# NVlabs/FB-BEV

Hardware: AMD Instinct MI355X
Metric: multi-cam samples/sec (forward view transformation: lift + voxel ranking + bev_pool_v2) (higher is better)
Workload: dtype f32

## Files before the change

fb_bev_amd/csrc/capi.hip:

```cpp
#include <stdio.h>
#include <stdlib.h>
#include <mutex>
#include "rt.h"
#include "pool_kernels.h"
#include "pool_bwd_kernels.h"
#include "rank_kernels.h"
#include "sort_kernels.h"
#include "msda_kernels.h"
#include "geom_kernels.h"
#include "da_kernels.h"
#include "history_kernels.h"
#include "norm_kernels.h"
#include "history_conv_kernels.h"
#include "history_fused_kernels.h"
#include "history_conv_x3_kernels.h"
#include "history_fused_x3_kernels.h"
#include "rows_linear_kernels.h"
#include "rows_linear_f32_kernels.h"
#include "da_fused_kernels.h"
#include "da_bwd_planes_kernels.h"
#include "msda_bwd_kernels.h"
#include "conv3d_kernels.h"
#include "det_kernels.h"
#include "occ_kernels.h"
// ... 29 lines not shown
}

extern "C" int fbbev_bev_pool_v2_bwd(int c, int n_intervals, const float* out_grad,
                                     const float* depth, const float* feat,
                                     const int32_t* ranks_depth, const int32_t* ranks_feat,
                                     const int32_t* ranks_bev, const int32_t* interval_starts,
                                     const int32_t* interval_lengths, float* depth_grad,
                                     float* feat_grad, fbbev_stream_t stream_) {
    if (c <= 0 || n_intervals < 0) return FBBEV_E_BADARG;
    if (c > 256) return FBBEV_E_UNSUPPORTED;
    if (n_intervals == 0) return 0;
    if (!out_grad || !depth || !feat || !ranks_depth || !ranks_feat || !ranks_bev ||
        !interval_starts || !interval_lengths || !depth_grad || !feat_grad) return FBBEV_E_BADARG;
    fbbev_rt_stream stream = (fbbev_rt_stream)stream_;
    const long long blocks = ((long long)n_intervals * 64 + 255) / 256;
    const int nch = (c + 63) / 64;
#define FBBEV_BWD(NCH)                                                                             \
    FBBEV_LAUNCH(k_pool_bwd<NCH>, blocks, 256, 0, stream, c, n_intervals, out_grad, depth, feat,   \
                 ranks_depth, ranks_feat, ranks_bev, interval_starts, interval_lengths, depth_grad, \
                 feat_grad)
    switch (nch) {
        case 1: FBBEV_BWD(1); break;
        case 2: FBBEV_BWD(2); break;
        case 3: FBBEV_BWD(3); break;
        default: FBBEV_BWD(4); break;
    }
#undef FBBEV_BWD
    FBBEV_CHECK_LAUNCH();
    return 0;
}

extern "C" int fbbev_lidar_coor(const float* xs, const float* ys, const float* ds, const float* rots,
                                const float* trans, const float* intrins, const float* post_rots,
                                const float* post_trans, const float* bda, int B, int N, int D, int H,
                                int W, float* coor, fbbev_stream_t stream_) {
    if (B <= 0 || N <= 0 || D <= 0 || H <= 0 || W <= 0) return FBBEV_E_BADARG;
    if (!xs || !ys || !ds || !rots || !trans || !intrins || !post_rots || !post_trans || !bda || !coor)
        return FBBEV_E_BADARG;
    const long long dhw = (long long)D * H * W;
    const long long chunks = (dhw + 255) / 256;
    if (chunks * B * N >= (1ll << 31)) return FBBEV_E_UNSUPPORTED;
    fbbev_cam_ptrs g;
    g.xs = xs; g.ys = ys; g.ds = ds; g.rots = rots; g.trans = trans; g.intrins = intrins; g.post_rots = post_rots;
    g.post_trans = post_trans; g.bda = bda; g.N = N; g.D = D; g.H = H; g.W = W;
    FBBEV_LAUNCH(k_lidar_coor, chunks * B * N, 256, 0, (fbbev_rt_stream)stream_, g, (int)chunks, coor);
    FBBEV_CHECK_LAUNCH();
    return 0;
}

extern "C" int fbbev_nchw_to_nhwc(const float* in, float* out, int n_images, int C, int HW, fbbev_stream_t stream_) {
    return fbbev_tokens_from_nchw(in, out, n_images, C, HW, (long long)C * HW, 0, nullptr, 0, stream_);
}

static int tokens_from_nchw_impl(const float* in, float* out, int n_images, int C, int HW, long long out_image_stride,
                                 long long out_offset, const float* bias, int bias_rows, const float* pos_bias,
                                 fbbev_stream_t stream_) {
    if (n_images < 0 || C <= 0 || HW <= 0 || out_offset < 0 || out_image_stride < (long long)C * HW) return FBBEV_E_BADARG;
    if (bias && bias_rows <= 0) return FBBEV_E_BADARG;
    if (n_images == 0) return 0;
    if (!in || !out) return FBBEV_E_BADARG;
    const int tc = (C + 31) / 32, th = (HW + 31) / 32;
    const long long blocks = (long long)n_images * tc * th;
    if (blocks >= (1ll << 31)) return FBBEV_E_UNSUPPORTED;
    FBBEV_LAUNCH(k_nchw_to_nhwc, blocks, 256, 0, (fbbev_rt_stream)stream_, in, out, C, HW, tc, th, out_image_stride,
                 out_offset, bias, bias ? bias_rows : 1, pos_bias);
    FBBEV_CHECK_LAUNCH();
    return 0;
}

extern "C" int fbbev_tokens_from_nchw(const float* in, float* out, int n_images, int C, int HW,
                                      long long out_image_stride, long long out_offset, const float* bias,
                                      int bias_rows, fbbev_stream_t stream_) {
    return tokens_from_nchw_impl(in, out, n_images, C, HW, out_image_stride, out_offset, bias, bias_rows, nullptr, stream_);
}

extern "C" int fbbev_tokens_from_nchw_levels(const float* const* in, const int32_t* hw, int n_levels, float* out, int n_images, int C,
                                             const float* bias, int bias_rows, fbbev_stream_t stream_) {
    if (n_levels <= 0 || n_levels > 8 || n_images < 0 || C <= 0 || !in || !hw) return FBBEV_E_BADARG;
    if (bias && bias_rows <= 0) return FBBEV_E_BADARG;
    if (n_images == 0) return 0;
    if (!out) return FBBEV_E_BADARG;
    fbbev_token_levels lv;
    const int tc = (C + 31) / 32;
    long long start = 0, blocks = 0;
    for (int l = 0; l < 8; ++l) { lv.in[l] = nullptr; lv.out_off[l] = 0; lv.hw[l] = 1; lv.blk0[l] = 0; }
    for (int l = 0; l < n_levels; ++l) {
        if (hw[l] <= 0 || !in[l]) return FBBEV_E_BADARG;
        lv.in[l] = in[l]; lv.hw[l] = hw[l]; lv.out_off[l] = start * C; lv.blk0[l] = (int)blocks;
        start += hw[l];
        blocks += (long long)n_images * tc * ((hw[l] + 31) / 32);
        if (blocks >= (1ll << 31)) return FBBEV_E_UNSUPPORTED;
    }
    lv.blk0[n_levels] = (int)blocks;
    lv.n = n_levels;
    FBBEV_LAUNCH(k_nchw_to_nhwc_levels, blocks, 256, 0, (fbbev_rt_stream)stream_, lv, out, C, tc, start * C, bias, bias ? bias_rows : 1);
    FBBEV_CHECK_LAUNCH();
    return 0;
}

extern "C" int fbbev_tokens_from_nchw_pos(const float* in, float* out, int n_images, int C, int HW, long long out_image_stride,
                                          long long out_offset, const float* pos_bias, fbbev_stream_t stream_) {
    if (!pos_bias) return FBBEV_E_BADARG;
    return tokens_from_nchw_impl(in, out, n_images, C, HW, out_image_stride, out_offset, nullptr, 0, pos_bias, stream_);
}

extern "C" int fbbev_point_sampling(const float* xs, const float* ys, const float* zs, const float* rots,
                                    const float* trans, const float* intrins, const float* post_rots,
                                    const float* post_trans, const float* bda, int B, int N, int Y, int X,
                                    int Za, float ogfH, float ogfW, float* ref_cam, uint8_t* mask,
                                    float* qdepth, fbbev_stream_t stream_) {
    if (B <= 0 || N <= 0 || Y <= 0 || X <= 0 || Za <= 0 || !(ogfH > 0.f) || !(ogfW > 0.f)) return FBBEV_E_BADARG;
    if (!xs || !ys || !zs || !rots || !trans || !intrins || !post_rots || !post_trans || !bda || !ref_cam ||
        !mask || !qdepth) return FBBEV_E_BADARG;
    const long long npts = (long long)Y * X * Za;
    int ppt = 8;
    while (ppt > 1 && (npts + 256 * ppt - 1) / (256 * ppt) * B * N < 1024) ppt >>= 1;
    const long long chunks = (npts + 256 * ppt - 1) / (256 * ppt);
    if (chunks * B * N >= (1ll << 31) || ((uintptr_t)ref_cam & 7) != 0) return FBBEV_E_UNSUPPORTED;
    FBBEV_LAUNCH(k_point_sampling, chunks * B * N, 256, 0, (fbbev_rt_stream)stream_, xs, ys, zs, rots, trans,
                 intrins, post_rots, post_trans, bda, B, N, Y, X, Za, ogfH, ogfW, (int)chunks, ref_cam, mask,
                 qdepth, ppt);
    FBBEV_CHECK_LAUNCH();
    return 0;
}

static inline int key_bits(long long total_voxels) {
    int bits = 1;
    while ((1ll << bits) < total_voxels) ++bits;
    return bits;
}

static const int kSortTile[7] = {2048, 4096, 8192, 12288, 16384, 4096, 8192};
static int sort_variant_for(long long items) {
    for (int v = 0; v < 5; ++v)
        if ((items + kSortTile[v] - 1) / kSortTile[v] <= 256) return v;
    return 6;
}
static const int kIvTile[3] = {1024, 4096, 8192};
static int iv_variant_for(long long items) {
    for (int v = 0; v < 3; ++v)
        if ((items + kIvTile[v] - 1) / kIvTile[v] <= 256) return v;
    return 2;
}

static fbbev_fastdiv make_fastdiv(unsigned int d) {
    fbbev_fastdiv f;
    f.d = d; f.m = 0; f.sh = 0;
    if (d <= 1) { f.d = 1; return f; }
    unsigned int l = 0;
    while ((1ull << l) < d) ++l;
    f.m = (unsigned int)((((1ull << l) - d) << 32) / d + 1);
    f.sh = l - 1;
    return f;
}

struct rank_ws_layout {
    size_t keys_a, keys_t, vals_t, matrix, ctot, chunk_info, boff, hb, total;
    int v0, wgs0;
    int v1, wgs1;
    int vi, wgsi;
};

static rank_ws_layout rank_layout(long long n) {
    rank_ws_layout L;
    L.v0 = sort_variant_for(n);
    L.v1 = sort_variant_for((n + 1) / 2);
    L.vi = iv_variant_for((n + 1) / 2);
    if (const char* env = fbbev_env_str("FBBEV_RANK_SHAPE")) {
        int a = -1, b = -1, c = -1;
        if (sscanf(env, "%d,%d,%d", &a, &b, &c) == 3 && a >= 0 && a < 7 && b >= 0 && b < 7 && c >= 0 && c < 3) {
            L.v0 = a; L.v1 = b; L.vi = c;
        }
    }
    L.wgs0 = (int)((n + kSortTile[L.v0] - 1) / kSortTile[L.v0]);
    L.wgs1 = (int)((n + kSortTile[L.v1] - 1) / kSortTile[L.v1]);
    L.wgsi = (int)((n + kIvTile[L.vi] - 1) / kIvTile[L.vi]);
    size_t off = 0;
    L.keys_a = off; off = align_up(off + (size_t)n * 4, 256);
    L.keys_t = off; off = align_up(off + (size_t)n * 4, 256);
    L.vals_t = off; off = align_up(off + (size_t)n * 4, 256);
    const int rows = L.wgs0 > L.wgs1 ? L.wgs0 : L.wgs1;
    const size_t seg_rows = (size_t)(n / FBBEV_SEG_TILE) + 256 + 1;
    size_t mbytes = (size_t)rows * FBBEV_SORT_MAX_NB * 4;
    if (seg_rows * FBBEV_SEG_NB * 4 > mbytes) mbytes = seg_rows * FBBEV_SEG_NB * 4;
    L.matrix = off; off = align_up(off + mbytes, 256);
    L.ctot = off; off = align_up(off + seg_rows * 4, 256);
    L.chunk_info = off; off = align_up(off + (size_t)L.wgsi * 8, 256);
    const size_t fin_buckets = (size_t)(n < 256 ? n : 256) * FBBEV_SEG_NB;
    L.boff = off; off = align_up(off + (fin_buckets + 1) * 4, 256);
    L.hb = off; off = align_up(off + fin_buckets * 4, 256);
    L.total = off;
    return L;
}

#define FBBEV_SORT_DISPATCH(KERNEL, v, by_waves, grid, stream, ...)                                             \
    do {                                                                                                        \
        switch (v) {                                                                                            \
            case 0: FBBEV_LAUNCH((KERNEL<(by_waves) ? 4 : 256, 8>), grid, 256, 0, stream, __VA_ARGS__); break;   \
            case 1: FBBEV_LAUNCH((KERNEL<(by_waves) ? 16 : 1024, 4>), grid, 1024, 0, stream, __VA_ARGS__); break; \
            case 2: FBBEV_LAUNCH((KERNEL<(by_waves) ? 16 : 1024, 8>), grid, 1024, 0, stream, __VA_ARGS__); break; \
            case 3: FBBEV_LAUNCH((KERNEL<(by_waves) ? 16 : 1024, 12>), grid, 1024, 0, stream, __VA_ARGS__); break; \
            case 5: FBBEV_LAUNCH((KERNEL<(by_waves) ? 8 : 512, 8>), grid, 512, 0, stream, __VA_ARGS__); break;     \
            case 6: FBBEV_LAUNCH((KERNEL<(by_waves) ? 8 : 512, 16>), grid, 512, 0, stream, __VA_ARGS__); break;    \
            default: FBBEV_LAUNCH((KERNEL<(by_waves) ? 16 : 1024, 16>), grid, 1024, 0, stream, __VA_ARGS__); break; \
        }                                                                                                       \
    } while (0)

extern "C" size_t fbbev_rank_workspace_bytes(int64_t n_points) {
    if (n_points <= 0) return 256;
    return rank_layout(n_points).total;
}

static int rank_seg_mode() { FBBEV_KNOB_ONCE(int, m, fbbev_env_int("FBBEV_RANK_SEG", -1)); return m; }
static int rank_finish_mode() { FBBEV_KNOB_ONCE(int, m, fbbev_env_int("FBBEV_RANK_FINISH", -1)); return m; }
static bool rank_finish_auto(int lbits, long long npb, int B) {
    (void)npb; (void)B;
    return lbits >= 2 * FBBEV_SEG_RB;
}

static int rank_build_impl(const float* coor, const fbbev_cam_ptrs* cams, const float* frustum, int B, int N, int D,
                           int H, int W,
                           const float* lower3, const float* interval3, const float* grid_size3,
                           int32_t* ranks_bev, int32_t* ranks_depth, int32_t* ranks_feat,
                           int32_t* interval_starts, int32_t* interval_lengths, int32_t* interval_rank,
                           int32_t* counts, void* workspace, size_t workspace_bytes, fbbev_rt_stream stream,
                           const float* point_depth = nullptr, float depth_thr = 0.f, const int* skip = nullptr) {
    if (B <= 0 || N <= 0 || D <= 0 || H <= 0 || W <= 0) return FBBEV_E_BADARG;
    if (point_depth && cams) return FBBEV_E_UNSUPPORTED;
    if ((!coor && !cams) || !lower3 || !interval3 || !grid_size3 || !ranks_bev || !ranks_depth || !ranks_feat ||
        !interval_starts || !interval_lengths || !counts || !workspace) return FBBEV_E_BADARG;
    const long long n = (long long)B * N * D * H * W;
    if (n >= (1ll << 30)) return FBBEV_E_UNSUPPORTED;
    const rank_ws_layout L = rank_layout(n);
    if (workspace_bytes < L.total) return FBBEV_E_WORKSPACE;
    unsigned char* ws = static_cast<unsigned char*>(workspace);
    unsigned int* keys_a = reinterpret_cast<unsigned int*>(ws + L.keys_a);
    unsigned int* keys_t = reinterpret_cast<unsigned int*>(ws + L.keys_t);
    unsigned int* vals_t = reinterpret_cast<unsigned int*>(ws + L.vals_t);
    int* matrix = reinterpret_cast<int*>(ws + L.matrix);
    int2* chunk_info = reinterpret_cast<int2*>(ws + L.chunk_info);

    fbbev_grid_params gp;
    gp.lx = lower3[0]; gp.ly = lower3[1]; gp.lz = lower3[2];
    gp.ix = interval3[0]; gp.iy = interval3[1]; gp.iz = interval3[2];
    gp.gx = grid_size3[0]; gp.gy = grid_size3[1]; gp.gz = grid_size3[2];
    volatile float zy = gp.gz * gp.gy;
    volatile float zyx = zy * gp.gx;
    volatile float yx = gp.gy * gp.gx;
    gp.f_zyx = zyx; gp.f_yx = yx;
    const long long total_voxels = (long long)B * (long long)gp.gz * (long long)gp.gy * (long long)gp.gx;
    if (total_voxels <= 0 || total_voxels >= (1ll << 30)) return FBBEV_E_UNSUPPORTED;
    const int bits = key_bits(total_voxels + 128);
    struct { int passes, rb; } plan;
    plan.passes = (bits + FBBEV_SORT_MAX_RB - 1) / FBBEV_SORT_MAX_RB;
    plan.rb = (bits + plan.passes - 1) / plan.passes;
    if (plan.rb < 4) plan.rb = 4;
    const int rb = plan.rb;
    const int seg_mode = rank_seg_mode();
    const long long vps = total_voxels / B;
    const long long npb = n / B;
    const int lbits = key_bits(vps);
    const bool seg_legal = B <= 256 && total_voxels <= (1ll << 24) && lbits <= 2 * FBBEV_SEG_RB;
    const long long seg_cps = (npb + FBBEV_SEG_TILE - 1) / FBBEV_SEG_TILE;
    const bool seg = seg_legal && seg_mode != 0 &&
                     (seg_mode == 2 || ((lbits + FBBEV_SEG_RB - 1) / FBBEV_SEG_RB < plan.passes && seg_cps <= 64 && B * seg_cps >= 96));
    if (seg) {
        fbbev_seg sg;
        sg.npb = (int)npb; sg.cps = (int)((npb + FBBEV_SEG_TILE - 1) / FBBEV_SEG_TILE); sg.vps = (unsigned int)vps; sg.nseg = B;
        const int passes = (lbits + FBBEV_SEG_RB - 1) / FBBEV_SEG_RB;
        const int srb = (lbits + passes - 1) / passes < 4 ? 4 : (lbits + passes - 1) / passes;
        const int wgs = B * sg.cps;
        int* ctot = reinterpret_cast<int*>(ws + L.ctot);
        fbbev_geom_src gs;
        if (cams) { gs.cam = *cams; gs.frustum = frustum; gs.gp = gp; }
        else { gs.cam = fbbev_cam_ptrs(); gs.frustum = nullptr; gs.gp = gp; }
        const int fin_mode = rank_finish_mode();
        const bool finish = passes == 2 && fin_mode != 0 && (fin_mode == 1 || rank_finish_auto(lbits, npb, B));
        const int high_bits = FBBEV_SEG_RB, low_bits = lbits - FBBEV_SEG_RB;
        const int rb0 = finish ? high_bits : srb, dshift0 = finish ? low_bits : 0;
        if (cams) FBBEV_LAUNCH((k_keys_hist_seg<true>), wgs, FBBEV_SEG_NT, 0, stream, gs, (const float*)nullptr, gp, (const float*)nullptr, 0.f,
                               sg, rb0, dshift0, skip, keys_a, matrix, ctot);
        else FBBEV_LAUNCH((k_keys_hist_seg<false>), wgs, FBBEV_SEG_NT, 0, stream, gs, coor, gp, point_depth, depth_thr, sg, rb0, dshift0, skip,
                          keys_a, matrix, ctot);
        FBBEV_CHECK_LAUNCH();
        if (finish) {
            int* boff = reinterpret_cast<int*>(ws + L.boff);
            int* hb = reinterpret_cast<int*>(ws + L.hb);
            const int nbk = (int)((vps + (1ll << low_bits) - 1) >> low_bits);
            const int buckets = B * nbk;
            static const int swz = fbbev_env_int("FBBEV_RANK_XCD_SWIZZLE", 1);
            const int sw = (swz && B >= 8) ? 1 : 0;
            FBBEV_LAUNCH(k_sort_scatter_seg, sw ? (wgs + 7) / 8 * 8 : wgs, FBBEV_SEG_NT, 0, stream, (const unsigned int*)keys_a,
                         (const unsigned int*)nullptr, (const int*)matrix, (const int*)ctot, sg, 0, high_bits, skip, keys_t, vals_t, counts, sw, 2,
                         low_bits, boff, nbk);
            FBBEV_CHECK_LAUNCH();
            const fbbev_fastdiv div_dhw = make_fastdiv((unsigned int)((long long)D * H * W)), div_hw = make_fastdiv((unsigned int)(H * W));
            int short_wgs = (buckets + FBBEV_FIN_WAVES - 1) / FBBEV_FIN_WAVES;
            if (short_wgs > 2048) short_wgs = 2048;
            const int long_wgs = buckets < 512 ? buckets : 512;
            FBBEV_LAUNCH(k_bucket_finish, long_wgs + short_wgs, FBBEV_FIN_WAVES * 64, 0, stream, reinterpret_cast<const uint2*>(keys_t),
                         (const int*)boff, buckets, nbk, sg.vps, low_bits, long_wgs, div_dhw, div_hw, skip,
                         reinterpret_cast<unsigned int*>(ranks_bev), reinterpret_cast<unsigned int*>(ranks_depth), ranks_feat, hb);
            FBBEV_CHECK_LAUNCH();
            const int per_wg = (buckets + 255) / 256;
            FBBEV_LAUNCH((k_bucket_intervals<16, 4>), (buckets + per_wg - 1) / per_wg, 1024, (size_t)2 * 4 * 1024 * 4, stream,
                         reinterpret_cast<const unsigned int*>(ranks_bev), (const int*)boff, (const int*)hb, buckets, per_wg, skip,
                         interval_starts, interval_lengths, interval_rank, counts);
            FBBEV_CHECK_LAUNCH();
            return 0;
        }
        const unsigned int* kin = keys_a;
        const unsigned int* vin = nullptr;
        static const int pairs = fbbev_env_int("FBBEV_RANK_PAIRS", 1);
        for (int p = 0; p < passes; ++p) {
            const bool to_out = p == passes - 1;
            const int pm = pairs ? ((p > 0 ? 1 : 0) | (to_out ? 0 : 2)) : 0;
            unsigned int* ko = to_out ? reinterpret_cast<unsigned int*>(ranks_bev) : keys_t;
            unsigned int* vo = to_out ? reinterpret_cast<unsigned int*>(ranks_depth) : vals_t;
            if (p > 0) {
                FBBEV_LAUNCH(k_sort_hist_seg, wgs, FBBEV_SEG_NT, 0, stream, kin, (const int*)ctot, sg, p * srb, srb, skip, matrix,
                             (pm & 1) ? 2 : 1);
                FBBEV_CHECK_LAUNCH();
            }
            static const int swz = fbbev_env_int("FBBEV_RANK_XCD_SWIZZLE", 1);
            const int sw = (swz && B >= 8) ? 1 : 0;
            FBBEV_LAUNCH(k_sort_scatter_seg, sw ? (wgs + 7) / 8 * 8 : wgs, FBBEV_SEG_NT, 0, stream, kin, vin, (const int*)matrix,
                         (const int*)ctot, sg, p, srb, skip, ko, vo, counts, sw, pm, -1, (int*)nullptr, 0);
            FBBEV_CHECK_LAUNCH();
            kin = ko; vin = vo;
        }
    } else {
    if (cams) {
            fbbev_geom_src gs;
            gs.cam = *cams; gs.frustum = frustum; gs.gp = gp;
            FBBEV_SORT_DISPATCH(k_keys_hist_geom, L.v0, false, L.wgs0, stream, gs, n, rb, skip, keys_a, matrix);
        } else {
            FBBEV_SORT_DISPATCH(k_keys_hist_coor, L.v0, false, L.wgs0, stream, coor, n, n / B, gp, point_depth, depth_thr, rb, keys_a, matrix);
        }
        FBBEV_CHECK_LAUNCH();
        const unsigned int* kin = keys_a;
        const unsigned int* vin = nullptr;
        for (int p = 0; p < plan.passes; ++p) {
            const bool to_out = ((plan.passes - 1 - p) % 2) == 0;
            unsigned int* ko = to_out ? reinterpret_cast<unsigned int*>(ranks_bev) : keys_t;
            unsigned int* vo = to_out ? reinterpret_cast<unsigned int*>(ranks_depth) : vals_t;
            const int v = p == 0 ? L.v0 : L.v1, wgs = p == 0 ? L.wgs0 : L.wgs1;
            if (p > 0) {
                FBBEV_SORT_DISPATCH(k_sort_hist, v, false, wgs, stream, kin, (const int*)counts, p * rb, rb, skip, matrix);
                FBBEV_CHECK_LAUNCH();
            }
            static const int swz = fbbev_env_int("FBBEV_RANK_XCD_SWIZZLE", 1);
            const bool sw = swz == 2 && p == 0;
            FBBEV_SORT_DISPATCH(k_sort_scatter, v, true, sw ? (wgs + 7) / 8 * 8 : wgs, stream, kin, vin, n, (const int*)matrix, p, rb, skip,
                                ko, vo, counts, sw ? wgs : 0);
            FBBEV_CHECK_LAUNCH();
            kin = ko; vin = vo;
        }
}
    const unsigned int* keys = reinterpret_cast<const unsigned int*>(ranks_bev);
    const unsigned int* vals = reinterpret_cast<const unsigned int*>(ranks_depth);
    const fbbev_fastdiv div_dhw = make_fastdiv((unsigned int)((long long)D * H * W)), div_hw = make_fastdiv((unsigned int)(H * W));
    switch (L.vi) {
        case 0:
            FBBEV_LAUNCH((k_interval_count<4, 4>), L.wgsi, 256, 0, stream, keys, (const int*)counts, skip, chunk_info);
            FBBEV_LAUNCH((k_interval_write<4, 4>), L.wgsi, 256, (size_t)2 * 4 * 256 * 4, stream, keys, vals, div_dhw, div_hw, (const int2*)chunk_info, skip,
                         ranks_feat, interval_starts, interval_lengths, interval_rank, counts);
            break;
        case 1:
            FBBEV_LAUNCH((k_interval_count<16, 4>), L.wgsi, 1024, 0, stream, keys, (const int*)counts, skip, chunk_info);
            FBBEV_LAUNCH((k_interval_write<16, 4>), L.wgsi, 1024, (size_t)2 * 4 * 1024 * 4, stream, keys, vals, div_dhw, div_hw, (const int2*)chunk_info, skip,
                         ranks_feat, interval_starts, interval_lengths, interval_rank, counts);
            break;
        default:
            FBBEV_LAUNCH((k_interval_count<16, 8>), L.wgsi, 1024, 0, stream, keys, (const int*)counts, skip, chunk_info);
            FBBEV_LAUNCH((k_interval_write<16, 8>), L.wgsi, 1024, (size_t)2 * 8 * 1024 * 4, stream, keys, vals, div_dhw, div_hw, (const int2*)chunk_info, skip,
                         ranks_feat, interval_starts, interval_lengths, interval_rank, counts);
            break;
    }
    FBBEV_CHECK_LAUNCH();
    return 0;
}

extern "C" int fbbev_rank_build(const float* coor, int B, int N, int D, int H, int W,
                                const float* lower3, const float* interval3,
                                const float* grid_size3, int32_t* ranks_bev, int32_t* ranks_depth,
                                int32_t* ranks_feat, int32_t* interval_starts,
                                int32_t* interval_lengths, int32_t* interval_rank, int32_t* counts,
                                void* workspace, size_t workspace_bytes, fbbev_stream_t stream_) {
    if (!coor) return FBBEV_E_BADARG;
    return rank_build_impl(coor, nullptr, nullptr, B, N, D, H, W, lower3, interval3, grid_size3, ranks_bev, ranks_depth,
                           ranks_feat, interval_starts, interval_lengths, interval_rank, counts, workspace,
                           workspace_bytes, (fbbev_rt_stream)stream_);
}

extern "C" int fbbev_rank_build_depth(const float* coor, const float* depth, float depth_threshold, int B, int N, int D,
                                      int H, int W, const float* lower3, const float* interval3,
                                      const float* grid_size3, int32_t* ranks_bev, int32_t* ranks_depth,
                                      int32_t* ranks_feat, int32_t* interval_starts, int32_t* interval_lengths,
                                      int32_t* interval_rank, int32_t* counts, void* workspace, size_t workspace_bytes,
                                      fbbev_stream_t stream_) {
    if (!coor || !depth) return FBBEV_E_BADARG;
    return rank_build_impl(coor, nullptr, nullptr, B, N, D, H, W, lower3, interval3, grid_size3, ranks_bev, ranks_depth,
                           ranks_feat, interval_starts, interval_lengths, interval_rank, counts, workspace,
                           workspace_bytes, (fbbev_rt_stream)stream_, depth, depth_threshold);
}

static int lift_rank_build_impl(const float* frustum, const float* xs, const float* ys, const float* ds,
                                const float* rots, const float* trans, const float* intrins, const float* post_rots,
                                const float* post_trans, const float* bda, int B, int N, int D, int H, int W,
                                const float* lower3, const float* interval3, const float* grid_size3,
                                int32_t* ranks_bev, int32_t* ranks_depth, int32_t* ranks_feat, int32_t* interval_starts,
                                int32_t* interval_lengths, int32_t* interval_rank, int32_t* counts, void* workspace,
                                size_t workspace_bytes, fbbev_rt_stream stream, uint32_t* cam_key, int32_t* cache_state) {
    if (!xs || !ys || !ds || !rots || !trans || !intrins || !post_rots || !post_trans || !bda) return FBBEV_E_BADARG;
    if (B <= 0 || N <= 0) return FBBEV_E_BADARG;
    fbbev_cam_ptrs g;
    g.xs = xs; g.ys = ys; g.ds = ds; g.rots = rots; g.trans = trans; g.intrins = intrins; g.post_rots = post_rots;
    g.post_trans = post_trans; g.bda = bda; g.N = N; g.D = D; g.H = H; g.W = W;
    const int* skip = nullptr;
    if (cam_key) {
        if (!cache_state) return FBBEV_E_BADARG;
        FBBEV_LAUNCH(k_cam_key, 1, 256, 0, stream, g, B, cam_key, cache_state);
        FBBEV_CHECK_LAUNCH();
        skip = cache_state;
    }
    return rank_build_impl(nullptr, &g, frustum, B, N, D, H, W, lower3, interval3, grid_size3, ranks_bev, ranks_depth,
                           ranks_feat, interval_starts, interval_lengths, interval_rank, counts, workspace,
                           workspace_bytes, stream, nullptr, 0.f, skip);
}

extern "C" int fbbev_lift_rank_build(const float* frustum, const float* xs, const float* ys, const float* ds,
                                     const float* rots,
                                     const float* trans, const float* intrins, const float* post_rots,
                                     const float* post_trans, const float* bda, int B, int N, int D, int H,
                                     int W, const float* lower3, const float* interval3,
                                     const float* grid_size3, int32_t* ranks_bev, int32_t* ranks_depth,
                                     int32_t* ranks_feat, int32_t* interval_starts, int32_t* interval_lengths,
                                     int32_t* interval_rank, int32_t* counts, void* workspace,
                                     size_t workspace_bytes, fbbev_stream_t stream_) {
    return lift_rank_build_impl(frustum, xs, ys, ds, rots, trans, intrins, post_rots, post_trans, bda, B, N, D, H, W, lower3,
                                interval3, grid_size3, ranks_bev, ranks_depth, ranks_feat, interval_starts,
                                interval_lengths, interval_rank, counts, workspace, workspace_bytes,
                                (fbbev_rt_stream)stream_, nullptr, nullptr);
}

extern "C" size_t fbbev_cam_key_words(int B, int N) {
    return (B <= 0 || N <= 0) ? 0 : (size_t)B * N * 33 + (size_t)B * 9;
}

extern "C" int fbbev_lift_rank_build_cached(const float* frustum, const float* xs, const float* ys, const float* ds,
                                            const float* rots, const float* trans, const float* intrins,
                                            const float* post_rots, const float* post_trans, const float* bda, int B,
                                            int N, int D, int H, int W, const float* lower3, const float* interval3,
                                            const float* grid_size3, int32_t* ranks_bev, int32_t* ranks_depth,
                                            int32_t* ranks_feat, int32_t* interval_starts, int32_t* interval_lengths,
                                            int32_t* interval_rank, int32_t* counts, void* workspace,
                                            size_t workspace_bytes, uint32_t* cam_key, int32_t* cache_state,
                                            fbbev_stream_t stream_) {
    if (!cam_key || !cache_state) return FBBEV_E_BADARG;
    return lift_rank_build_impl(frustum, xs, ys, ds, rots, trans, intrins, post_rots, post_trans, bda, B, N, D, H, W, lower3,
                                interval3, grid_size3, ranks_bev, ranks_depth, ranks_feat, interval_starts,
                                interval_lengths, interval_rank, counts, workspace, workspace_bytes,
                                (fbbev_rt_stream)stream_, cam_key, cache_state);
}

static inline int pick_tile(int tile_voxels) {
    switch (tile_voxels) { case 64: case 128: case 256: case 512: case 1024: return tile_voxels; default: return 64; }
}
static inline int small_tile_shift(int tile_voxels) {
    switch (tile_voxels) { case 8: return 3; case 16: return 4; case 32: return 5; default: return 0; }
}

extern "C" size_t fbbev_pool_dense_workspace_bytes(int B, int Z, int Y, int X) {
    if (B <= 0 || Z <= 0 || Y <= 0 || X <= 0) return 256;
    const long long yx = (long long)Y * X;
    const long long tiles = ((long long)B * Z * yx + 7) / 8 + (long long)B * Z;
    return align_up((size_t)(tiles + 2) * 8, 256);
}

static int pool_tile_index_impl(const int32_t* interval_rank, const int32_t* interval_starts,
                                const int32_t* counts, int n_intervals_max, int B, int Z, int Y,
                                int X, int tile_voxels, int flags, void* tile_ws, size_t tile_ws_bytes,
                                fbbev_stream_t stream_, const int32_t* skip);

extern "C" int fbbev_pool_tile_index(const int32_t* interval_rank, const int32_t* interval_starts,
                                     const int32_t* counts, int n_intervals_max, int B, int Z, int Y,
                                     int X, int tile_voxels, int flags, void* tile_ws, size_t tile_ws_bytes,
                                     fbbev_stream_t stream_) {
    return pool_tile_index_impl(interval_rank, interval_starts, counts, n_intervals_max, B, Z, Y, X, tile_voxels, flags,
                                tile_ws, tile_ws_bytes, stream_, nullptr);
}

extern "C" int fbbev_pool_tile_index_cached(const int32_t* interval_rank, const int32_t* interval_starts,
                                            const int32_t* counts, int n_intervals_max, int B, int Z, int Y,
                                            int X, int tile_voxels, int flags, void* tile_ws, size_t tile_ws_bytes,
                                            const int32_t* cache_state, int32_t* table_gate,
                                            fbbev_stream_t stream_) {
    if (!cache_state || !table_gate) return FBBEV_E_BADARG;
    if ((flags & FBBEV_POOL_CHANNELS_LAST) && small_tile_shift(tile_voxels)) return FBBEV_E_UNSUPPORTED;
    FBBEV_LAUNCH(k_tile_table_gate, 1, 1, 0, (fbbev_rt_stream)stream_, cache_state, table_gate);
    FBBEV_CHECK_LAUNCH();
    return pool_tile_index_impl(interval_rank, interval_starts, counts, n_intervals_max, B, Z, Y, X, tile_voxels, flags,
                                tile_ws, tile_ws_bytes, stream_, table_gate + 1);
}

static int pool_tile_index_impl(const int32_t* interval_rank, const int32_t* interval_starts,
                                const int32_t* counts, int n_intervals_max, int B, int Z, int Y,
                                int X, int tile_voxels, int flags, void* tile_ws, size_t tile_ws_bytes,
                                fbbev_stream_t stream_, const int32_t* skip) {
    if (B <= 0 || Z <= 0 || Y <= 0 || X <= 0 || n_intervals_max < 0) return FBBEV_E_BADARG;
    if (!interval_rank || !interval_starts || !counts || !tile_ws) return FBBEV_E_BADARG;
    const long long yx = (long long)Y * X;
    if ((long long)B * Z * yx >= (1ll << 31)) return FBBEV_E_UNSUPPORTED;
    if ((flags & FBBEV_POOL_CHANNELS_LAST) && small_tile_shift(tile_voxels)) {
        const int sh = small_tile_shift(tile_voxels);
        const long long nvox = (long long)B * Z * yx;
        const long long nt = (nvox + (1 << sh) - 1) >> sh;
        if (tile_ws_bytes < (size_t)nt * 8) return FBBEV_E_WORKSPACE;
        int* first = static_cast<int*>(tile_ws);
        int e = fbbev_rt_memset_async(first, 0xFF, (size_t)nt * 8, (fbbev_rt_stream)stream_);
        if (e) return e;
        long long blocks = ((long long)n_intervals_max + 255) / 256;
        if (blocks > 4096) blocks = 4096;
        if (blocks < 1) blocks = 1;
        FBBEV_LAUNCH(k_tile_scatter, blocks, 256, 0, (fbbev_rt_stream)stream_, interval_rank, counts,
                     n_intervals_max, sh, nvox, first, first + nt);
        FBBEV_CHECK_LAUNCH();
        return 0;
    }
    const int TV = pick_tile(tile_voxels);
    int tiles_per_plane = (int)((yx + TV - 1) / TV);
    long long n_tiles = (long long)B * Z * tiles_per_plane;
    long long plane = yx;
    if (flags & FBBEV_POOL_CHANNELS_LAST) {
        plane = (long long)B * Z * yx;
        n_tiles = (plane + TV - 1) / TV;
        tiles_per_plane = (int)n_tiles + 1;
    }
    if (tile_ws_bytes < (size_t)(n_tiles + 1) * 8) return FBBEV_E_WORKSPACE;
    FBBEV_LAUNCH(k_tile_lower_bound2, (n_tiles + 1 + 255) / 256, 256, 0, (fbbev_rt_stream)stream_,
                 (int)n_tiles, tiles_per_plane, (int)plane, TV, interval_rank, interval_starts, counts,
                 n_intervals_max, skip, static_cast<int*>(tile_ws));
    FBBEV_CHECK_LAUNCH();
    return 0;
}

struct dense2_args {
    long long n_blocks; size_t lds; fbbev_rt_stream stream; int C, Z, yx, tpp, csplit, swizzle;
    long long stride_b, stride_c;
    const float *depth, *feat; const int32_t *rd, *rf, *irank, *starts, *lengths; const int* tile_meta;
    const float* addend = nullptr;
    float* out;
    bool split = false;
    bool gather8 = false;
};

#define FBBEV_POOL_SPLIT_LEN 32
template <int TV, int CPL, int ST, int NT, int OT, bool T16 = false, int SPLIT = 0, int GU = 4>
static int launch_dense2(const dense2_args& a) {
    size_t lds = a.lds;
    if (SPLIT > 0) lds += ((size_t)TV + 4) * sizeof(int) + (size_t)FBBEV_POOL_SPLIT_GROUPS * (a.C / a.csplit) * sizeof(float);
    if (T16)
        lds = (size_t)(a.C / a.csplit) * (TV + 8) * 2 + ((size_t)3 * TV + 2 * FBBEV_NP_STAGE) * sizeof(int);
    long long grid = a.n_blocks;
    if (a.swizzle) {
        const long long g = 8ll << (a.swizzle - 1);
        grid = (a.n_blocks + g - 1) / g * g;
    }
    FBBEV_LAUNCH_DYN_LDS((k_pool_fwd_dense2<TV, CPL, ST, NT, OT, T16, 0, SPLIT, GU>), grid, NT, lds, a.stream, a.C, a.Z, a.yx, a.tpp,
                         a.csplit, (int)a.n_blocks, a.swizzle, a.stride_b, a.stride_c, a.depth, a.feat, a.rd, a.rf, a.irank, a.starts, a.lengths, a.tile_meta, a.addend, a.out);
    return fbbev_rt_last_error();
}

template <int TV, int CPL, int ST>
static int launch_dense2_nt(int nt, int ot, const dense2_args& a) {
    if (a.split) {
        if constexpr (ST == 4 && (TV == 64 || TV == 128)) {
            if (ot == 0 && nt == 256) return launch_dense2<TV, CPL, 4, 256, 0, false, FBBEV_POOL_SPLIT_LEN>(a);
        }
        return FBBEV_E_UNSUPPORTED;
    }
    if (a.gather8) {
        if constexpr (ST == 4 && (TV == 64 || TV == 128)) {
            if (ot == 0 && nt == 256) return launch_dense2<TV, CPL, 4, 256, 0, false, 0, 8>(a);
        }
        return FBBEV_E_UNSUPPORTED;
    }
    if constexpr (ST == 4) {
        if (ot != 0 && !a.addend && nt == 256)
            return ot == 1 ? launch_dense2<TV, CPL, 4, 256, 1, true>(a) : launch_dense2<TV, CPL, 4, 256, 2, true>(a);
        if (ot == 1) return nt == 128 ? launch_dense2<TV, CPL, 4, 128, 1>(a) : launch_dense2<TV, CPL, 4, 256, 1>(a);
        if (ot == 2) return nt == 128 ? launch_dense2<TV, CPL, 4, 128, 2>(a) : launch_dense2<TV, CPL, 4, 256, 2>(a);
    }
    return nt == 128 ? launch_dense2<TV, CPL, ST, 128, 0>(a) : launch_dense2<TV, CPL, ST, 256, 0>(a);
}

template <int TV, int CPL, int ST, int NT>
static int launch_dense_cl(const dense2_args& a) {
    long long grid = a.n_blocks;
    if (a.swizzle) {
        const long long g = 8ll << (a.swizzle - 1);
        grid = (a.n_blocks + g - 1) / g * g;
    }
    FBBEV_LAUNCH((k_pool_fwd_dense_cl<TV, CPL, ST, NT>), grid, NT, a.lds, a.stream, a.C, a.yx, (int)a.n_blocks,
                 a.swizzle, a.depth, a.feat, a.rd, a.rf, a.irank, a.starts, a.lengths, a.tile_meta, a.out);
    return fbbev_rt_last_error();
}

template <int TV, int CPL>
// ... 3184 lines not shown
```

fb_bev_amd/csrc/rank_kernels.h:

```cpp
#pragma once
#include "rt.h"


struct fbbev_grid_params {
    float lx, ly, lz;
    float ix, iy, iz;
    float gx, gy, gz;
    float f_yx, f_zyx;
};

__device__ __forceinline__ unsigned int fbbev_rank_key(float cx, float cy, float cz, const fbbev_grid_params& gp,
                                                       float bf, unsigned int sentinel) {
    const float fx = __fdiv_rn(fbbev_sub(cx, gp.lx), gp.ix);
    const float fy = __fdiv_rn(fbbev_sub(cy, gp.ly), gp.iy);
    const float fz = __fdiv_rn(fbbev_sub(cz, gp.lz), gp.iz);
    const bool finite = (fx == fx) && (fy == fy) && (fz == fz) && fabsf(fx) < 2.0e9f &&
                        fabsf(fy) < 2.0e9f && fabsf(fz) < 2.0e9f;
    const int vx = finite ? (int)fx : -1;
    const int vy = finite ? (int)fy : -1;
    const int vz = finite ? (int)fz : -1;
    const bool kept = finite && vx >= 0 && vy >= 0 && vz >= 0 && (float)vx < gp.gx &&
                      (float)vy < gp.gy && (float)vz < gp.gz;
    float r = fbbev_mul(bf, gp.f_zyx);
    r = fbbev_add(r, fbbev_mul((float)vz, gp.f_yx));
    const float t = fbbev_add(fbbev_mul((float)vy, gp.gx), (float)vx);
    r = fbbev_add(r, t);
    return kept ? (unsigned int)(int)r : sentinel;
}

__device__ __forceinline__ int fbbev_wave_incl_scan(int v, int lane) {
#pragma unroll
    for (int o = 1; o < 64; o <<= 1) {
        const int n = __shfl_up(v, o, 64);
        if (lane >= o) v += n;
    }
    return v;
}

__device__ __forceinline__ int fbbev_block_excl_scan(int v, int* lds4, int* total) {
    const int lane = threadIdx.x & 63, w = threadIdx.x >> 6;
    const int inc = fbbev_wave_incl_scan(v, lane);
    if (lane == 63) lds4[w] = inc;
    __syncthreads();
    int woff = 0, tot = 0;
#pragma unroll
    for (int i = 0; i < 4; ++i) {
        const int x = lds4[i];
        if (i < w) woff += x;
        tot += x;
    }
    __syncthreads();
    *total = tot;
    return woff + inc - v;
}

template <int WAVES, bool MAX>
__device__ __forceinline__ int fbbev_block_excl_scan_w(int v, int* ldsw, int* total) {
    const int lane = threadIdx.x & 63, w = threadIdx.x >> 6;
    int inc = v;
#pragma unroll
    for (int o = 1; o < 64; o <<= 1) {
        const int nbr = __shfl_up(inc, o, 64);
        if (lane >= o) inc = MAX ? (nbr > inc ? nbr : inc) : inc + nbr;
    }
    int excl = __shfl_up(inc, 1, 64);
    if (lane == 0) excl = 0;
    if (lane == 63) ldsw[w] = inc;
    __syncthreads();
    int carry = 0, tot = 0;
#pragma unroll
    for (int i = 0; i < WAVES; ++i) {
        const int x = ldsw[i];
        if (i < w) carry = MAX ? (x > carry ? x : carry) : carry + x;
        tot = MAX ? (x > tot ? x : tot) : tot + x;
    }
    __syncthreads();
    *total = tot;
    return MAX ? (excl > carry ? excl : carry) : carry + excl;
}

template <int ITEMS>
__device__ __forceinline__ void fbbev_ld_run(const unsigned int* __restrict__ p, long long base, long long P, unsigned int fill,
                                             unsigned int (&r)[ITEMS]) {
    static_assert(ITEMS % 4 == 0, "runs of whole 16-byte groups");
    if (base + ITEMS <= P && ((reinterpret_cast<uintptr_t>(p + base) & 15u) == 0)) {
#pragma unroll
        for (int q = 0; q < ITEMS / 4; ++q) {
            const fbbev_v4u t = *reinterpret_cast<const fbbev_v4u*>(p + base + 4 * q);
            r[4 * q] = t[0]; r[4 * q + 1] = t[1]; r[4 * q + 2] = t[2]; r[4 * q + 3] = t[3];
        }
    } else {
#pragma unroll
        for (int j = 0; j < ITEMS; ++j) r[j] = (base + j < P) ? p[base + j] : fill;
    }
}

template <int WAVES, int ITEMS>
__global__ void __launch_bounds__(WAVES * 64)
k_interval_count(const unsigned int* __restrict__ keys, const int* __restrict__ counts, const int* __restrict__ skip,
                 int2* __restrict__ chunk_info) {
    if (skip != nullptr && *skip != 0) return;
    constexpr int NT = WAVES * 64;
    constexpr int TILE = NT * ITEMS;
    __shared__ int ldsw[WAVES];
    const int tid = threadIdx.x;
    const int P = counts[0];
    const long long wg0 = (long long)blockIdx.x * TILE;
    if (wg0 >= P) return;
    const long long base = wg0 + (long long)tid * ITEMS;
    int local = 0, last1 = 0;
    unsigned int prevk = (base > 0 && base <= P) ? keys[base - 1] : 0u;
    unsigned int kk[ITEMS];
    fbbev_ld_run<ITEMS>(keys, base, P, 0u, kk);
#pragma unroll
    for (int j = 0; j < ITEMS; ++j) {
        const long long i = base + j;
        if (i < P) {
            const unsigned int k = kk[j];
            if (i == 0 || prevk != k) { ++local; last1 = (int)i + 1; }
            prevk = k;
        }
    }
    int tot, wg_last1;
    (void)fbbev_block_excl_scan_w<WAVES, false>(local, ldsw, &tot);
    (void)fbbev_block_excl_scan_w<WAVES, true>(last1, ldsw, &wg_last1);
    if (tid == 0) chunk_info[blockIdx.x] = make_int2(tot, wg_last1);
}

struct fbbev_fastdiv { unsigned int d, m, sh; };
__device__ __forceinline__ unsigned int fbbev_div(unsigned int n, const fbbev_fastdiv& f) {
    if (f.d == 1u) return n;
    const unsigned int t = (unsigned int)(((unsigned long long)n * f.m) >> 32);
    return (t + ((n - t) >> 1)) >> f.sh;
}

template <int WAVES, int ITEMS>
__global__ void __launch_bounds__(WAVES * 64)
k_interval_write(const unsigned int* __restrict__ keys, const unsigned int* __restrict__ vals, fbbev_fastdiv div_dhw,
                 fbbev_fastdiv div_hw, const int2* __restrict__ chunk_info, const int* __restrict__ skip, int* __restrict__ ranks_feat,
                 int* __restrict__ interval_starts, int* __restrict__ interval_lengths, int* __restrict__ interval_rank,
                 int* __restrict__ counts) {
    if (skip != nullptr && *skip != 0) return;
    constexpr int NT = WAVES * 64;
    constexpr int TILE = NT * ITEMS;
    __shared__ int ldsw[WAVES];
    const int tid = threadIdx.x;
    const int wg = blockIdx.x;
    const int P = counts[0];
    const long long wg0 = (long long)wg * TILE;
    if (wg0 >= P) {
        if (wg == 0 && tid == 0) counts[1] = 0;
        return;
    }
    int h = 0, l1 = 0;
    for (int r = tid; r < wg; r += NT) {
        const int2 ci = chunk_info[r];
        h += ci.x;
        l1 = ci.y > l1 ? ci.y : l1;
    }
    int before_heads, before_last1;
    (void)fbbev_block_excl_scan_w<WAVES, false>(h, ldsw, &before_heads);
    (void)fbbev_block_excl_scan_w<WAVES, true>(l1, ldsw, &before_last1);
    const long long base = wg0 + (long long)tid * ITEMS;
    bool head[ITEMS];
    unsigned int key[ITEMS];
    int local = 0, last1 = 0;
    unsigned int prevk = (base > 0 && base <= P) ? keys[base - 1] : 0u;
    unsigned int pid[ITEMS];
    fbbev_ld_run<ITEMS>(keys, base, P, 0u, key);
    fbbev_ld_run<ITEMS>(vals, base, P, 0u, pid);
    int rf[ITEMS];
#pragma unroll
    for (int j = 0; j < ITEMS; ++j) {
        const long long i = base + j;
        head[j] = false;
        rf[j] = 0;
        if (i < P) {
            const unsigned int k = key[j];
            head[j] = (i == 0 || prevk != k);
            prevk = k;
            if (head[j]) { ++local; last1 = (int)i + 1; }
            const unsigned int cam = fbbev_div(pid[j], div_dhw), hw = pid[j] - fbbev_div(pid[j], div_hw) * div_hw.d;
            rf[j] = (int)(cam * div_hw.d + hw);
        }
    }
    if (base + ITEMS <= P && ((reinterpret_cast<uintptr_t>(ranks_feat + base) & 15u) == 0)) {
#pragma unroll
        for (int q = 0; q < ITEMS / 4; ++q) {
            fbbev_v4i t;
            t[0] = rf[4 * q]; t[1] = rf[4 * q + 1]; t[2] = rf[4 * q + 2]; t[3] = rf[4 * q + 3];
            *reinterpret_cast<fbbev_v4i*>(ranks_feat + base + 4 * q) = t;
        }
    } else {
#pragma unroll
        for (int j = 0; j < ITEMS; ++j)
            if (base + j < P) ranks_feat[base + j] = rf[j];
    }
    int tot, wg_last1;
    const int off = fbbev_block_excl_scan_w<WAVES, false>(local, ldsw, &tot);
    (void)fbbev_block_excl_scan_w<WAVES, true>(last1, ldsw, &wg_last1);
    int* hpos = reinterpret_cast<int*>(fbbev_dyn_lds_f32());
    int* hkey = hpos + TILE;
    {
        int o = off;
#pragma unroll
        for (int j = 0; j < ITEMS; ++j)
            if (head[j]) { hpos[o] = (int)(base + j); hkey[o] = (int)key[j]; ++o; }
    }
    __syncthreads();
    for (int o = tid; o < tot; o += NT) {
        const int pos = hpos[o], j0 = before_heads + o;
        interval_starts[j0] = pos;
        if (interval_rank) interval_rank[j0] = hkey[o];
        if (j0 > 0) interval_lengths[j0 - 1] = pos - (o > 0 ? hpos[o - 1] : before_last1 - 1);
    }
    if (tid == 0 && wg0 + TILE >= P) {
        const int I = before_heads + tot;
        const int lasthead1 = wg_last1 ? wg_last1 : before_last1;
        interval_lengths[I - 1] = P - (lasthead1 - 1);
        counts[1] = I;
    }
}

template <int WAVES, int ITEMS>
__global__ void __launch_bounds__(WAVES * 64)
k_bucket_intervals(const unsigned int* __restrict__ keys, const int* __restrict__ boff, const int* __restrict__ hb, int buckets,
                   int per_wg, const int* __restrict__ skip, int* __restrict__ interval_starts, int* __restrict__ interval_lengths,
                   int* __restrict__ interval_rank, int* __restrict__ counts) {
    if (skip != nullptr && *skip != 0) return;
    constexpr int NT = WAVES * 64;
    constexpr int TILE = NT * ITEMS;
    __shared__ int ldsw[WAVES];
    const int tid = threadIdx.x;
    const int g0 = (int)blockIdx.x * per_wg;
    if (g0 >= buckets) return;
    const int g1 = g0 + per_wg < buckets ? g0 + per_wg : buckets;
    const int r0 = boff[g0], r1 = boff[g1];
    int h = 0;
    {
        constexpr int U = 4;
        const int nq = g0 >> 2;
        const fbbev_v4i* hb4 = reinterpret_cast<const fbbev_v4i*>(hb);
        for (int q0 = tid; q0 < nq; q0 += NT * U) {
            fbbev_v4i t[U];
#pragma unroll
            for (int u = 0; u < U; ++u) {
                const int qi = q0 + u * NT;
                t[u] = hb4[qi < nq ? qi : nq - 1];
            }
#pragma unroll
            for (int u = 0; u < U; ++u)
                if (q0 + u * NT < nq) h += t[u][0] + t[u][1] + t[u][2] + t[u][3];
        }
        if (tid < (g0 & 3)) h += hb[4 * nq + tid];
    }
    int hbase;
    (void)fbbev_block_excl_scan_w<WAVES, false>(h, ldsw, &hbase);
    int* hpos = reinterpret_cast<int*>(fbbev_dyn_lds_f32());
    int* hkey = hpos + TILE;
    int lastpos = r0;
    for (int t0 = r0; t0 < r1; t0 += TILE) {
        const long long base = (long long)t0 + (long long)tid * ITEMS;
        bool head[ITEMS];
        unsigned int key[ITEMS];
        int local = 0;
        unsigned int prevk = (base > r0 && base <= r1) ? keys[base - 1] : 0u;
        fbbev_ld_run<ITEMS>(keys, base, r1, 0u, key);
#pragma unroll
        for (int j = 0; j < ITEMS; ++j) {
            const long long i = base + j;
            head[j] = false;
            if (i < r1) {
                head[j] = (i == r0 || prevk != key[j]);
                prevk = key[j];
                if (head[j]) ++local;
            }
        }
        int tot;
        int o = fbbev_block_excl_scan_w<WAVES, false>(local, ldsw, &tot);
#pragma unroll
        for (int j = 0; j < ITEMS; ++j)
            if (head[j]) { hpos[o] = (int)(base + j); hkey[o] = (int)key[j]; ++o; }
        __syncthreads();
        for (int q = tid; q < tot; q += NT) {
            const int pos = hpos[q], j0 = hbase + q;
            interval_starts[j0] = pos;
            if (interval_rank) interval_rank[j0] = hkey[q];
            if (q > 0) interval_lengths[j0 - 1] = pos - hpos[q - 1];
            else if (t0 > r0) interval_lengths[j0 - 1] = pos - lastpos;
        }
        if (tot > 0) lastpos = hpos[tot - 1];
        hbase += tot;
        __syncthreads();
    }
    if (tid == 0) {
        if (r1 > r0) interval_lengths[hbase - 1] = r1 - lastpos;
        if (g1 == buckets) counts[1] = hbase;
    }
}
```

Measured before the change: 23660.

## Partition bucket interval extraction by point ranges instead of bucket counts

The interval-building kernel now gives each workgroup a fixed range of sorted points (R elements) rather than a fixed number of buckets. Each workgroup finds the bucket boundaries snapping to its range and the head-count prefix by scanning all bucket offsets. This balances the load when bucket sizes are skewed. Other changes: block shape goes to 8 waves by 8 items, heads are tracked as a bitmask with popcount, and index math uses 32-bit ints. The cost is that every workgroup now reads the whole boff and hb arrays, and the grid can grow to up to 1024 workgroups.

```diff
diff --git a/fb_bev_amd/csrc/capi.hip b/fb_bev_amd/csrc/capi.hip
--- a/fb_bev_amd/csrc/capi.hip
+++ b/fb_bev_amd/csrc/capi.hip
@@ -355,9 +355,10 @@
                          (const int*)boff, buckets, nbk, sg.vps, low_bits, long_wgs, div_dhw, div_hw, skip,
                          reinterpret_cast<unsigned int*>(ranks_bev), reinterpret_cast<unsigned int*>(ranks_depth), ranks_feat, hb);
             FBBEV_CHECK_LAUNCH();
-            const int per_wg = (buckets + 255) / 256;
-            FBBEV_LAUNCH((k_bucket_intervals<16, 4>), (buckets + per_wg - 1) / per_wg, 1024, (size_t)2 * 4 * 1024 * 4, stream,
-                         reinterpret_cast<const unsigned int*>(ranks_bev), (const int*)boff, (const int*)hb, buckets, per_wg, skip,
+            const int iv_r = n <= (long long)FBBEV_IV_R * FBBEV_IV_MAX_WGS ? FBBEV_IV_R
+                                                                           : (int)((n + FBBEV_IV_MAX_WGS - 1) / FBBEV_IV_MAX_WGS + 3) / 4 * 4;
+            FBBEV_LAUNCH((k_bucket_intervals<8, 8>), (n + iv_r - 1) / iv_r, 512, (size_t)2 * 8 * 512 * 4, stream,
+                         reinterpret_cast<const unsigned int*>(ranks_bev), (const int*)boff, (const int*)hb, buckets, iv_r, skip,
                          interval_starts, interval_lengths, interval_rank, counts);
             FBBEV_CHECK_LAUNCH();
             return 0;
diff --git a/fb_bev_amd/csrc/rank_kernels.h b/fb_bev_amd/csrc/rank_kernels.h
--- a/fb_bev_amd/csrc/rank_kernels.h
+++ b/fb_bev_amd/csrc/rank_kernels.h
@@ -222,79 +222,111 @@
     }
 }
 
+#define FBBEV_IV_R 2048
+#define FBBEV_IV_MAX_WGS 1024
 template <int WAVES, int ITEMS>
 __global__ void __launch_bounds__(WAVES * 64)
 k_bucket_intervals(const unsigned int* __restrict__ keys, const int* __restrict__ boff, const int* __restrict__ hb, int buckets,
-                   int per_wg, const int* __restrict__ skip, int* __restrict__ interval_starts, int* __restrict__ interval_lengths,
+                   int R, const int* __restrict__ skip, int* __restrict__ interval_starts, int* __restrict__ interval_lengths,
                    int* __restrict__ interval_rank, int* __restrict__ counts) {
     if (skip != nullptr && *skip != 0) return;
     constexpr int NT = WAVES * 64;
     constexpr int TILE = NT * ITEMS;
-    __shared__ int ldsw[WAVES];
-    const int tid = threadIdx.x;
-    const int g0 = (int)blockIdx.x * per_wg;
-    if (g0 >= buckets) return;
-    const int g1 = g0 + per_wg < buckets ? g0 + per_wg : buckets;
-    const int r0 = boff[g0], r1 = boff[g1];
-    int h = 0;
+    static_assert(TILE >= 64 + WAVES && 3 * WAVES <= 64, "the reduction words live in front of the compacted heads");
+    const int tid = threadIdx.x, lane = tid & 63, wv = tid >> 6;
+    int* hpos = reinterpret_cast<int*>(fbbev_dyn_lds_f32());
+    int* hkey = hpos + TILE;
+    int* red = hpos;
+    int* ldsw = hpos + 64;
+    const bool last = blockIdx.x + 1 == gridDim.x;
+    const int P = boff[buckets];
+    const int lo = (int)blockIdx.x * R;
+    if (lo >= P && !last) return;
+    const int hi = last ? 0x7fffffff : lo + R;
+    int h = 0, r0 = P, r1 = P;
     {
-        constexpr int U = 4;
-        const int nq = g0 >> 2;
+        constexpr int U = 3;
+        const int nq = buckets >> 2;
         const fbbev_v4i* hb4 = reinterpret_cast<const fbbev_v4i*>(hb);
+        const fbbev_v4i* bo4 = reinterpret_cast<const fbbev_v4i*>(boff);
         for (int q0 = tid; q0 < nq; q0 += NT * U) {
-            fbbev_v4i t[U];
+            fbbev_v4i tb[U], th[U];
 #pragma unroll
             for (int u = 0; u < U; ++u) {
                 const int qi = q0 + u * NT;
-                t[u] = hb4[qi < nq ? qi : nq - 1];
+                tb[u] = bo4[qi < nq ? qi : nq - 1];
+                th[u] = hb4[qi < nq ? qi : nq - 1];
             }
 #pragma unroll
             for (int u = 0; u < U; ++u)
-                if (q0 + u * NT < nq) h += t[u][0] + t[u][1] + t[u][2] + t[u][3];
-        }
-        if (tid < (g0 & 3)) h += hb[4 * nq + tid];
-    }
-    int hbase;
-    (void)fbbev_block_excl_scan_w<WAVES, false>(h, ldsw, &hbase);
-    int* hpos = reinterpret_cast<int*>(fbbev_dyn_lds_f32());
-    int* hkey = hpos + TILE;
+                if (q0 + u * NT < nq) {
+#pragma unroll
+                    for (int e = 0; e < 4; ++e) {
+                        const int b = tb[u][e];
+                        if (b < lo) h += th[u][e]; else r0 = b < r0 ? b : r0;
+                        if (b >= hi) r1 = b < r1 ? b : r1;
+                    }
+                }
+        }
+        if (tid < (buckets & 3)) {
+            const int b = boff[4 * nq + tid];
+            if (b < lo) h += hb[4 * nq + tid]; else r0 = b < r0 ? b : r0;
+            if (b >= hi) r1 = b < r1 ? b : r1;
+        }
+    }
+#pragma unroll
+    for (int o = 32; o > 0; o >>= 1) {
+        h += __shfl_xor(h, o, 64);
+        const int a = __shfl_xor(r0, o, 64), b = __shfl_xor(r1, o, 64);
+        r0 = a < r0 ? a : r0;
+        r1 = b < r1 ? b : r1;
+    }
+    if (lane == 0) { red[3 * wv] = h; red[3 * wv + 1] = r0; red[3 * wv + 2] = r1; }
+    __syncthreads();
+    int hbase = 0;
+#pragma unroll 4
+    for (int i = 0; i < WAVES; ++i) {
+        const int a = red[3 * i + 1], b = red[3 * i + 2];
+        hbase += red[3 * i];
+        r0 = a < r0 ? a : r0;
+        r1 = b < r1 ? b : r1;
+    }
     int lastpos = r0;
-    for (int t0 = r0; t0 < r1; t0 += TILE) {
-        const long long base = (long long)t0 + (long long)tid * ITEMS;
-        bool head[ITEMS];
+    bool first = true;
+    for (int t0 = r0 & ~3; t0 < r1; t0 += TILE) {
+        const int base = t0 + tid * ITEMS;
         unsigned int key[ITEMS];
-        int local = 0;
+        unsigned int heads = 0;
         unsigned int prevk = (base > r0 && base <= r1) ? keys[base - 1] : 0u;
         fbbev_ld_run<ITEMS>(keys, base, r1, 0u, key);
 #pragma unroll
         for (int j = 0; j < ITEMS; ++j) {
-            const long long i = base + j;
-            head[j] = false;
-            if (i < r1) {
-                head[j] = (i == r0 || prevk != key[j]);
+            const int i = base + j;
+            if (i >= r0 && i < r1) {
+                if (i == r0 || prevk != key[j]) heads |= 1u << j;
                 prevk = key[j];
-                if (head[j]) ++local;
             }
         }
         int tot;
-        int o = fbbev_block_excl_scan_w<WAVES, false>(local, ldsw, &tot);
+        int o = fbbev_block_excl_scan_w<WAVES, false>(__popcll((unsigned long long)heads), ldsw, &tot);
 #pragma unroll
         for (int j = 0; j < ITEMS; ++j)
-            if (head[j]) { hpos[o] = (int)(base + j); hkey[o] = (int)key[j]; ++o; }
+            if (heads >> j & 1u) { hpos[o] = base + j; hkey[o] = (int)key[j]; ++o; }
         __syncthreads();
         for (int q = tid; q < tot; q += NT) {
             const int pos = hpos[q], j0 = hbase + q;
             interval_starts[j0] = pos;
             if (interval_rank) interval_rank[j0] = hkey[q];
             if (q > 0) interval_lengths[j0 - 1] = pos - hpos[q - 1];
-            else if (t0 > r0) interval_lengths[j0 - 1] = pos - lastpos;
+            else if (!first) interval_lengths[j0 - 1] = pos - lastpos;
         }
         if (tot > 0) lastpos = hpos[tot - 1];
         hbase += tot;
+        first = false;
         __syncthreads();
     }
     if (tid == 0) {
         if (r1 > r0) interval_lengths[hbase - 1] = r1 - lastpos;
-        if (g1 == buckets) counts[1] = hbase;
-    }
-}
+        if (last) counts[1] = hbase;
+    }
+}
```

Result: no change. 23780 (median of 5 runs) (+0.5%).
